# regicide211212/multi-style-transfer-gan

Hardware: AMD Instinct MI355X
Metric: train-step images/sec (fwd+bwd+loss), 256x256 batch32 (higher is better)
Workload: dtype f32; 1 GPU; config 3: reference CycleGAN train_step (2x EnhancedGenerator + 2x EnhancedDiscriminator, channels=16, num_transformer_blocks=0), 32 image pairs/GPU at 256x256, fwd+bwd+loss+Adam; per_gpu_batch=32, size=256, channels=16, parallelism=dp1, collective=none, losses_finite=True

## Files before the change

multi-style-transfer-gan_amd/mstg_hip/csrc/common.h:

```cpp
#pragma once
#include <hip/hip_runtime.h>
#include <stdint.h>
#include <stdio.h>
#include <string.h>

#include "mstg_hip.h"

typedef float f32x4 __attribute__((ext_vector_type(4)));
typedef float f32x2 __attribute__((ext_vector_type(2)));

namespace mstg {

extern thread_local char g_last_error[256];
inline int fail_launch(hipError_t e, const char* what) {
    snprintf(g_last_error, sizeof(g_last_error), "%s: %s", what, hipGetErrorString(e));
    return MSTG_E_LAUNCH;
}
inline int fail_arg(int code, const char* what) {
    snprintf(g_last_error, sizeof(g_last_error), "%s", what);
    return code;
}
#define MSTG_CHECK_LAUNCH(what)                                   \
    do {                                                          \
        hipError_t e__ = hipGetLastError();                       \
        if (e__ != hipSuccess) return mstg::fail_launch(e__, what); \
    } while (0)

extern bool g_prof_on;
void prof_begin(const void* host_fn, hipStream_t st);
void prof_end(hipStream_t st);
#define MSTG_LAUNCH(kern, grid, block, lds, st, ...)                               \
    do {                                                                           \
        const bool prof__ = mstg::g_prof_on;                                       \
        if (prof__) mstg::prof_begin((const void*)(kern), (hipStream_t)(st));      \
        hipLaunchKernelGGL(kern, grid, block, lds, st, __VA_ARGS__);               \
        if (prof__) mstg::prof_end((hipStream_t)(st));                             \
    } while (0)

extern thread_local bool t_ws_packed;
#define MSTG_PACK_LAUNCH(...)                      \
    do {                                           \
        if (!mstg::t_ws_packed) MSTG_LAUNCH(__VA_ARGS__); \
    } while (0)

enum EnvKnob {
    ENV_ATTN_BLK4, ENV_ATTN_BLK64, ENV_WGRAD_1X1, ENV_WGRAD_TS_MAXCH, ENV_WGRAD_PLAIN, ENV_WGRAD_OLD, ENV_NO_DPACK, ENV_IGEMM,
    ENV_STREAM, ENV_PF, ENV_WGLOB, ENV_HEAVY_PER_CU, ENV_DBG, ENV_DBG_LDS_KB, ENV_MS_WGRAD_PACKED, ENV_MS_FWD4, ENV_NO_PACK_CACHE,
    ENV_P32, ENV_P32_TH, ENV_P32_WLDS, ENV_P32_DBG, ENV_P32_OCC, ENV_ATTN_REG, ENV_NFW_ADAPT, ENV_BSUMS_ALL, ENV_ATTN_BIG32, ENV_NORM_WGS,
    ENV_CONV_IMG, ENV_COUNT
};
const char* env_get(EnvKnob k);

int cu_count();
struct OccCache {
    const void* kern = nullptr;
    size_t lds = 0;
    int occ = 1;
};
int persistent_occupancy(OccCache& c, const void* kern, size_t lds);

constexpr int WAVE = 64;

__device__ __forceinline__ f32x4 mfma16(float a, float b, f32x4 c) {
    return __builtin_amdgcn_mfma_f32_16x16x4f32(a, b, c, 0, 0, 0);
}

__device__ __forceinline__ float wave_sum(float v) {
#pragma unroll
    for (int o = 32; o > 0; o >>= 1) v += __shfl_xor(v, o, 64);
    return v;
}

__device__ __forceinline__ float apply_act(float v, int act) {
    switch (act) {
        case MSTG_ACT_RELU: return v > 0.f ? v : 0.f;
        case MSTG_ACT_LEAKY02: return v > 0.f ? v : 0.2f * v;
        case MSTG_ACT_TANH: return tanhf(v);
        case MSTG_ACT_GELU: return 0.5f * v * (1.f + erff(v * 0.70710678118654752f));
        default: return v;
    }
}
__device__ __forceinline__ float act_grad(float v, int act) {
    switch (act) {
        case MSTG_ACT_RELU: return v > 0.f ? 1.f : 0.f;
        case MSTG_ACT_LEAKY02: return v > 0.f ? 1.f : 0.2f;
        case MSTG_ACT_TANH: return 1.f - v * v;
        case MSTG_ACT_GELU: return 0.5f * (1.f + erff(v * 0.70710678118654752f)) + v * 0.3989422804014327f * expf(-0.5f * v * v);
        default: return 1.f;
    }
}

__device__ __forceinline__ int xcd_swizzle(int bid, int nblk) {
    const int q = nblk >> 3, r = nblk & 7, xcd = bid & 7, k = bid >> 3;
    return (xcd < r ? xcd * (q + 1) : r * (q + 1) + (xcd - r) * q) + k;
}


__host__ __device__ __forceinline__ unsigned magic_u32(unsigned d) { return 0xFFFFFFFFu / d + 1u; }

template <int NB>
__device__ __forceinline__ void stage_window_batch(const float* __restrict__ img, float* __restrict__ lds, int total, int e0, int cols,
                                                   int nq, unsigned m_cols, unsigned m_nq, int y0, int x0, int H, int W, int ctot,
                                                   int nq_valid, int ckp, int tid, int rowpad) {
    f32x4 v[NB];
    int dst[NB];
    bool ok[NB];
#pragma unroll
    for (int k = 0; k < NB; ++k) {
        const int e = e0 + 256 * k + tid;
        const int p = nq == 1 ? e : (int)__umulhi((unsigned)e, m_nq);
        const int q = e - p * nq;
        const int r = (int)__umulhi((unsigned)p, m_cols), c = p - r * cols;
        const int iy = y0 + r, ix = x0 + c;
        ok[k] = e < total && (unsigned)iy < (unsigned)H && (unsigned)ix < (unsigned)W && q < nq_valid;
        const unsigned off = ok[k] ? (unsigned)(iy * W + ix) * (unsigned)ctot + 4u * q : 0u;
        v[k] = *reinterpret_cast<const f32x4*>(img + off);
        dst[k] = e < total ? p * ckp + 4 * q + r * rowpad : -1;
    }
#pragma unroll
    for (int k = 0; k < NB; ++k)
        if (dst[k] >= 0) *reinterpret_cast<f32x4*>(&lds[dst[k]]) = ok[k] ? v[k] : f32x4{0.f, 0.f, 0.f, 0.f};
}

__device__ __forceinline__ void stage_window(const float* __restrict__ img, float* __restrict__ lds, int rows, int cols, int nq,
                                             unsigned m_cols, unsigned m_nq, int y0, int x0, int H, int W, int ctot, int nq_valid,
                                             int ckp, int tid, int rowpad = 0) {
    const int total = rows * cols * nq;
    int e0 = 0;
    for (; e0 + 1024 < total; e0 += 2048)
        stage_window_batch<8>(img, lds, total, e0, cols, nq, m_cols, m_nq, y0, x0, H, W, ctot, nq_valid, ckp, tid, rowpad);
    for (; e0 < total; e0 += 1024)
        stage_window_batch<4>(img, lds, total, e0, cols, nq, m_cols, m_nq, y0, x0, H, W, ctot, nq_valid, ckp, tid, rowpad);
}

__device__ __forceinline__ void stage_window_c4(const float* __restrict__ img, float* __restrict__ lds, int rows, int cols,
                                                unsigned m_cols, int y0, int x0, int H, int W, unsigned sy, unsigned sx, unsigned sc,
                                                int nch, int tid) {
    const int total = rows * cols;
    for (int e0 = 0; e0 < total; e0 += 1024) {
        f32x4 v[4];
        bool ok[4];
#pragma unroll
        for (int k = 0; k < 4; ++k) {
            const int e = e0 + 256 * k + tid;
            const int r = (int)__umulhi((unsigned)e, m_cols), c = e - r * cols;
            const int iy = y0 + r, ix = x0 + c;
            ok[k] = e < total && (unsigned)iy < (unsigned)H && (unsigned)ix < (unsigned)W;
            const unsigned off = ok[k] ? (unsigned)iy * sy + (unsigned)ix * sx : 0u;
#pragma unroll
            for (int ch = 0; ch < 4; ++ch) v[k][ch] = img[off + (ch < nch ? ch * sc : 0u)];
        }
#pragma unroll
        for (int k = 0; k < 4; ++k) {
            const int e = e0 + 256 * k + tid;
            if (e < total) {
                f32x4 w = {0.f, 0.f, 0.f, 0.f};
#pragma unroll
                for (int ch = 0; ch < 4; ++ch)
                    if (ok[k] && ch < nch) w[ch] = v[k][ch];
                *reinterpret_cast<f32x4*>(&lds[e * 4]) = w;
            }
        }
    }
}

inline int cdiv(int a, int b) { return (a + b - 1) / b; }
inline size_t cdivz(size_t a, size_t b) { return (a + b - 1) / b; }

}
```

multi-style-transfer-gan_amd/mstg_hip/csrc/norm.hip:

```cpp
#include "common.h"
#include <stdlib.h>

namespace mstg {

constexpr float NORM_EPS = 1e-5f;

struct NormGeom {
    int N, HW, C, split, chunk;
};

static NormGeom norm_geom(int N, int HW, int C) {
    NormGeom g;
    g.N = N; g.HW = HW; g.C = C;
    int wgs = 1024;
    { const char* e = env_get(ENV_NORM_WGS); if (e && atoi(e) >= 64) wgs = atoi(e); }
    int split = wgs / (N > 0 ? N : 1);
    if (split < 1) split = 1;
    const int maxsplit = cdiv(HW, 256);
    if (split > maxsplit) split = maxsplit;
    g.chunk = cdiv(HW, split);
    g.split = cdiv(HW, g.chunk);
    return g;
}

template <bool BWD>
__global__ __launch_bounds__(256) void norm_partial_kernel(const float* __restrict__ x, const float* __restrict__ dy,
                                                           const float* __restrict__ stats, const float* __restrict__ gamma,
                                                           const float* __restrict__ beta, float* __restrict__ partial,
                                                           NormGeom g, int act, int batch) {
    extern __shared__ __attribute__((aligned(16))) float red[];
    const int C = g.C, C4 = C >> 2, rows = 256 / C4;
    const int sp = blockIdx.x, n = blockIdx.y, tid = threadIdx.x;
    const int q = tid % C4, row = tid / C4;
    const int p0 = sp * g.chunk, p1 = min(g.HW, p0 + g.chunk);
    const float* xb = x + (size_t)n * g.HW * C;
    f32x4 s1 = {0.f, 0.f, 0.f, 0.f}, s2 = {0.f, 0.f, 0.f, 0.f};
    if (row < rows) {
        if (!BWD) {
            const f32x4 K = *reinterpret_cast<const f32x4*>((batch ? x : xb) + 4 * q);
            int p = p0 + row;
            constexpr int PX = 8;
            for (; p + (PX - 1) * rows < p1; p += PX * rows) {
                f32x4 v[PX];
#pragma unroll
                for (int k = 0; k < PX; ++k) v[k] = *reinterpret_cast<const f32x4*>(xb + (size_t)(p + k * rows) * C + 4 * q);
#pragma unroll
                for (int k = 0; k < PX; ++k) {
                    const f32x4 w = v[k] - K;
                    s1 += w;
                    s2 += w * w;
                }
            }
            for (; p < p1; p += rows) {
                const f32x4 v = *reinterpret_cast<const f32x4*>(xb + (size_t)p * C + 4 * q) - K;
                s1 += v;
                s2 += v * v;
            }
        } else {
            const float* st = stats + (size_t)(batch ? 0 : n) * C * 2;
            f32x4 mu, rs, ga = {1.f, 1.f, 1.f, 1.f}, be = {0.f, 0.f, 0.f, 0.f};
#pragma unroll
            for (int e = 0; e < 4; ++e) { mu[e] = st[(4 * q + e) * 2]; rs[e] = st[(4 * q + e) * 2 + 1]; }
            if (batch) { ga = *reinterpret_cast<const f32x4*>(gamma + 4 * q); be = *reinterpret_cast<const f32x4*>(beta + 4 * q); }
            const float* dyb = dy + (size_t)n * g.HW * C;
            int p = p0 + row;
            constexpr int PX = 8;
            for (; p + (PX - 1) * rows < p1; p += PX * rows) {
                f32x4 xv[PX], gv[PX];
#pragma unroll
                for (int k = 0; k < PX; ++k) {
                    xv[k] = *reinterpret_cast<const f32x4*>(xb + (size_t)(p + k * rows) * C + 4 * q);
                    gv[k] = *reinterpret_cast<const f32x4*>(dyb + (size_t)(p + k * rows) * C + 4 * q);
                }
#pragma unroll
                for (int k = 0; k < PX; ++k) {
                    const f32x4 xh = (xv[k] - mu) * rs;
                    f32x4 gg = gv[k];
#pragma unroll
                    for (int e = 0; e < 4; ++e) gg[e] *= act_grad(xh[e] * ga[e] + be[e], act);
                    s1 += gg;
                    s2 += gg * xh;
                }
            }
            for (; p < p1; p += rows) {
                const f32x4 xh = (*reinterpret_cast<const f32x4*>(xb + (size_t)p * C + 4 * q) - mu) * rs;
                f32x4 gg = *reinterpret_cast<const f32x4*>(dyb + (size_t)p * C + 4 * q);
#pragma unroll
                for (int e = 0; e < 4; ++e) gg[e] *= act_grad(xh[e] * ga[e] + be[e], act);
                s1 += gg;
                s2 += gg * xh;
            }
        }
        *reinterpret_cast<f32x4*>(&red[(row * 2 + 0) * C + 4 * q]) = s1;
        *reinterpret_cast<f32x4*>(&red[(row * 2 + 1) * C + 4 * q]) = s2;
    }
    __syncthreads();
    for (int e = tid; e < 2 * C; e += 256) {
        float acc = 0.f;
        for (int r = 0; r < rows; ++r) acc += red[r * 2 * C + e];
        partial[((size_t)n * g.split + sp) * 2 * C + e] = acc;
    }
}

template <bool BWD>
__global__ __launch_bounds__(256) void norm_apply_kernel(const float* __restrict__ x, const float* __restrict__ dy,
                                                         const float* __restrict__ residual, float* __restrict__ out,
                                                         float* __restrict__ stats, const float* __restrict__ gamma,
                                                         const float* __restrict__ beta, float* __restrict__ running_mean,
                                                         float* __restrict__ running_var, float* __restrict__ dgamma,
                                                         float* __restrict__ dbeta, const float* __restrict__ partial,
                                                         NormGeom g, int act, int batch, int psplit) {
    extern __shared__ __attribute__((aligned(16))) float sm[];
    const int C = g.C, C4 = C >> 2, rows = 256 / C4;
    const int sp = blockIdx.x, n = blockIdx.y, tid = threadIdx.x;
    const float cnt = batch ? (float)g.N * (float)g.HW : (float)g.HW;
    for (int c = tid; c < C; c += 256) {
        float t1 = 0.f, t2 = 0.f;
        if (batch != 2 && batch != 3) {
            const int nb = batch ? 0 : n, ne = batch ? g.N : n + 1;
            for (int nn = nb; nn < ne; ++nn) {
                const float* pp = partial + (size_t)nn * psplit * 2 * C + c;
                int s = 0;
                for (; s + 8 <= psplit; s += 8) {
                    float a[8], b[8];
#pragma unroll
                    for (int k = 0; k < 8; ++k) {
                        a[k] = pp[(size_t)(s + k) * 2 * C];
                        b[k] = pp[(size_t)(s + k) * 2 * C + C];
                    }
#pragma unroll
                    for (int k = 0; k < 8; ++k) {
                        t1 += a[k];
                        t2 += b[k];
                    }
                }
                for (; s < psplit; ++s) {
                    t1 += pp[(size_t)s * 2 * C];
                    t2 += pp[(size_t)s * 2 * C + C];
                }
            }
        }
        if (!BWD) {
            float mean, rstd;
            if (batch == 2) {
                mean = running_mean[c];
                rstd = rsqrtf(running_var[c] + NORM_EPS);
            } else if (batch == 3) {
                mean = stats[((size_t)n * C + c) * 2];
                rstd = stats[((size_t)n * C + c) * 2 + 1];
            } else {
                const float K = (batch ? x : x + (size_t)n * g.HW * C)[c];
                const float e1 = t1 / cnt;
                float var = t2 / cnt - e1 * e1;
                var = var > 0.f ? var : 0.f;
                mean = K + e1;
                rstd = rsqrtf(var + NORM_EPS);
                if (batch == 1 && sp == 0 && n == 0) {
                    running_mean[c] = 0.9f * running_mean[c] + 0.1f * mean;
                    running_var[c] = 0.9f * running_var[c] + 0.1f * var * (cnt / fmaxf(cnt - 1.f, 1.f));
                }
            }
            if (batch != 3 && sp == 0 && (!batch || n == 0)) {
                stats[((size_t)(batch ? 0 : n) * C + c) * 2] = mean;
                stats[((size_t)(batch ? 0 : n) * C + c) * 2 + 1] = rstd;
            }
            const bool affine = batch == 1 || batch == 2;
            const float ga = affine ? gamma[c] : 1.f, be = affine ? beta[c] : 0.f;
            sm[c] = rstd * ga;
            sm[C + c] = be;
            sm[2 * C + c] = mean;
        } else {
            const float* st = stats + (size_t)(batch ? 0 : n) * C * 2;
            const float mu = st[c * 2], rs = st[c * 2 + 1];
            const float ga = batch ? gamma[c] : 1.f;
            const float m1 = batch == 2 ? 0.f : t1 / cnt, m2 = batch == 2 ? 0.f : t2 / cnt;
            if (batch == 1 && sp == 0 && n == 0) { dgamma[c] = t2; dbeta[c] = t1; }
            sm[c] = mu;
            sm[C + c] = rs;
            sm[2 * C + c] = m1;
            sm[3 * C + c] = m2;
            (void)ga;
        }
    }
    __syncthreads();
    const int q = tid % C4, row = tid / C4;
    if (row >= rows) return;
    const int p0 = sp * g.chunk, p1 = min(g.HW, p0 + g.chunk);
    const size_t base = (size_t)n * g.HW * C;
    if (!BWD) {
        const f32x4 A = *reinterpret_cast<const f32x4*>(&sm[4 * q]), B = *reinterpret_cast<const f32x4*>(&sm[C + 4 * q]);
        const f32x4 M = *reinterpret_cast<const f32x4*>(&sm[2 * C + 4 * q]);
        int p = p0 + row;
        constexpr int PX = 8;
        for (; p + (PX - 1) * rows < p1; p += PX * rows) {
            f32x4 v[PX], r[PX];
#pragma unroll
            for (int k = 0; k < PX; ++k) {
                const size_t o = base + (size_t)(p + k * rows) * C + 4 * q;
                v[k] = __builtin_nontemporal_load(reinterpret_cast<const f32x4*>(x + o));
                if (residual) r[k] = __builtin_nontemporal_load(reinterpret_cast<const f32x4*>(residual + o));
            }
#pragma unroll
            for (int k = 0; k < PX; ++k) {
                const size_t o = base + (size_t)(p + k * rows) * C + 4 * q;
                f32x4 w = (v[k] - M) * A + B;
#pragma unroll
                for (int e = 0; e < 4; ++e) w[e] = apply_act(w[e], act);
                if (residual) w += r[k];
                *reinterpret_cast<f32x4*>(out + o) = w;
            }
        }
        for (; p < p1; p += rows) {
            const size_t o = base + (size_t)p * C + 4 * q;
            f32x4 v = (*reinterpret_cast<const f32x4*>(x + o) - M) * A + B;
#pragma unroll
            for (int e = 0; e < 4; ++e) v[e] = apply_act(v[e], act);
            if (residual) v += *reinterpret_cast<const f32x4*>(residual + o);
            *reinterpret_cast<f32x4*>(out + o) = v;
        }
    } else {
        const f32x4 mu = *reinterpret_cast<const f32x4*>(&sm[4 * q]), rs = *reinterpret_cast<const f32x4*>(&sm[C + 4 * q]);
        const f32x4 m1 = *reinterpret_cast<const f32x4*>(&sm[2 * C + 4 * q]), m2 = *reinterpret_cast<const f32x4*>(&sm[3 * C + 4 * q]);
        f32x4 ga = {1.f, 1.f, 1.f, 1.f}, be = {0.f, 0.f, 0.f, 0.f};
        if (batch) { ga = *reinterpret_cast<const f32x4*>(gamma + 4 * q); be = *reinterpret_cast<const f32x4*>(beta + 4 * q); }
        int p = p0 + row;
        constexpr int PX = 8;
        for (; p + (PX - 1) * rows < p1; p += PX * rows) {
            f32x4 xv[PX], gv[PX];
#pragma unroll
            for (int k = 0; k < PX; ++k) {
                const size_t o = base + (size_t)(p + k * rows) * C + 4 * q;
                xv[k] = __builtin_nontemporal_load(reinterpret_cast<const f32x4*>(x + o));
                gv[k] = __builtin_nontemporal_load(reinterpret_cast<const f32x4*>(dy + o));
            }
#pragma unroll
            for (int k = 0; k < PX; ++k) {
                const size_t o = base + (size_t)(p + k * rows) * C + 4 * q;
                const f32x4 xh = (xv[k] - mu) * rs;
                f32x4 gg = gv[k];
#pragma unroll
                for (int e = 0; e < 4; ++e) gg[e] *= act_grad(xh[e] * ga[e] + be[e], act);
                *reinterpret_cast<f32x4*>(out + o) = rs * ga * (gg - m1 - xh * m2);
            }
        }
        for (; p < p1; p += rows) {
            const size_t o = base + (size_t)p * C + 4 * q;
            const f32x4 xh = (*reinterpret_cast<const f32x4*>(x + o) - mu) * rs;
            f32x4 gg = *reinterpret_cast<const f32x4*>(dy + o);
#pragma unroll
            for (int e = 0; e < 4; ++e) gg[e] *= act_grad(xh[e] * ga[e] + be[e], act);
            *reinterpret_cast<f32x4*>(out + o) = rs * ga * (gg - m1 - xh * m2);
        }
    }
}

__device__ __forceinline__ void norm_row_sums(const float* __restrict__ partial, int n, int split, int C, int groups, float* red, float& t1,
                                              float& t2) {
    const int tid = threadIdx.x, c = tid % C, grp = tid / C;
    t1 = t2 = 0.f;
    if (grp < groups) {
        const float* pp = partial + (size_t)n * split * 2 * C + c;
        int s = grp;
        for (; s + 7 * groups < split; s += 8 * groups) {
            float a[8], b[8];
#pragma unroll
            for (int k = 0; k < 8; ++k) {
                a[k] = pp[(size_t)(s + k * groups) * 2 * C];
                b[k] = pp[(size_t)(s + k * groups) * 2 * C + C];
            }
#pragma unroll
            for (int k = 0; k < 8; ++k) {
                t1 += a[k];
                t2 += b[k];
            }
        }
        for (; s < split; s += groups) {
            t1 += pp[(size_t)s * 2 * C];
            t2 += pp[(size_t)s * 2 * C + C];
        }
    }
    if (groups > 1) {
        if (grp < groups) {
            red[(grp * 2 + 0) * C + c] = t1;
            red[(grp * 2 + 1) * C + c] = t2;
        }
        __syncthreads();
        if (grp == 0) {
            t1 = t2 = 0.f;
            for (int k = 0; k < groups; ++k) {
                t1 += red[(k * 2 + 0) * C + c];
                t2 += red[(k * 2 + 1) * C + c];
            }
        }
    }
}

static int norm_groups(const NormGeom& g) { return g.split > 32 && g.C <= 128 ? 256 / g.C : 1; }
static int norm_row_threads(const NormGeom& g) { const int t = g.C * norm_groups(g); return t < 64 ? 64 : ((t + 63) / 64) * 64; }

__global__ void norm_stats_kernel(const float* __restrict__ x, const float* __restrict__ partial, float* __restrict__ stats, NormGeom g,
                                  int groups) {
    extern __shared__ __attribute__((aligned(16))) float red[];
    const int n = blockIdx.x, C = g.C;
    const float cnt = (float)g.HW;
    float t1, t2;
    norm_row_sums(partial, n, g.split, C, groups, red, t1, t2);
    if ((int)threadIdx.x < C) {
        const int c = threadIdx.x;
        const float K = x[(size_t)n * g.HW * C + c];
        const float e1 = t1 / cnt;
        float var = t2 / cnt - e1 * e1;
        var = var > 0.f ? var : 0.f;
        stats[((size_t)n * C + c) * 2] = K + e1;
        stats[((size_t)n * C + c) * 2 + 1] = rsqrtf(var + NORM_EPS);
    }
}

__global__ void norm_sums_kernel(const float* __restrict__ partial, float* __restrict__ sums, NormGeom g, int groups) {
    extern __shared__ __attribute__((aligned(16))) float red[];
    const int n = blockIdx.x, C = g.C;
    float t1, t2;
    norm_row_sums(partial, n, g.split, C, groups, red, t1, t2);
    if ((int)threadIdx.x < C) {
        sums[((size_t)n * 2 + 0) * C + threadIdx.x] = t1;
        sums[((size_t)n * 2 + 1) * C + threadIdx.x] = t2;
    }
}

static int norm_check(int N, int HW, int C) {
    if (N <= 0 || HW <= 0 || C <= 0) return fail_arg(MSTG_E_BADARG, "norm: empty tensor");
    if (C % 4 || C > 1024) return fail_arg(MSTG_E_ALIGN, "norm: C must be a multiple of 4 and <= 1024");
    return MSTG_OK;
}

}

using namespace mstg;

extern "C" size_t mstg_norm_workspace_bytes(int N, int HW, int C) {
    if (N <= 0 || HW <= 0 || C <= 0) return 0;
    const NormGeom g = norm_geom(N, HW, C);
    return ((size_t)N * g.split * 2 * C + (size_t)N * 2 * C) * sizeof(float);
}

extern "C" int mstg_norm_act_fwd(const float* x, const float* residual, float* y, float* stats, int N, int HW, int C, int act,
                                 int batch_stats, const float* gamma, const float* beta, float* running_mean,
                                 float* running_var, void* workspace, size_t workspace_bytes, void* stream) {
    if (int rc = norm_check(N, HW, C)) return rc;
    if (!x || !y || !stats || !workspace) return fail_arg(MSTG_E_BADARG, "norm_fwd: null pointer");
    if (batch_stats && (!gamma || !beta || !running_mean || !running_var)) return fail_arg(MSTG_E_BADARG, "norm_fwd: batch norm needs gamma/beta/running stats");
    if (act == MSTG_ACT_TANH) return fail_arg(MSTG_E_UNSUPPORTED, "norm_fwd: tanh epilogue not supported");
    const NormGeom g = norm_geom(N, HW, C);
    if (workspace_bytes < mstg_norm_workspace_bytes(N, HW, C)) return fail_arg(MSTG_E_WORKSPACE, "norm_fwd: workspace too small");
    hipStream_t st = (hipStream_t)stream;
    const int rows = 256 / (C / 4);
    dim3 grid(g.split, N);
    if (batch_stats != 2) {
        MSTG_LAUNCH((norm_partial_kernel<false>), grid, dim3(256), (size_t)rows * 2 * C * sizeof(float), st, x, nullptr, nullptr,
                           gamma, beta, (float*)workspace, g, act, batch_stats);
        MSTG_CHECK_LAUNCH("norm_partial_kernel");
    }
    if (batch_stats == 0 && g.split > 32) {
        const int groups = norm_groups(g);
        MSTG_LAUNCH(norm_stats_kernel, dim3(N), dim3(norm_row_threads(g)), (size_t)groups * 2 * C * sizeof(float), st, x,
                    (const float*)workspace, stats, g, groups);
        MSTG_CHECK_LAUNCH("norm_stats_kernel");
        MSTG_LAUNCH((norm_apply_kernel<false>), grid, dim3(256), (size_t)4 * C * sizeof(float), st, x, nullptr, residual, y, stats, nullptr,
                    nullptr, nullptr, nullptr, nullptr, nullptr, nullptr, g, act, 3, 0);
        MSTG_CHECK_LAUNCH("norm_apply_kernel");
        return MSTG_OK;
    }
    MSTG_LAUNCH((norm_apply_kernel<false>), grid, dim3(256), (size_t)4 * C * sizeof(float), st, x, nullptr, residual, y, stats,
                       gamma, beta, running_mean, running_var, nullptr, nullptr, (const float*)workspace, g, act, batch_stats, g.split);
    MSTG_CHECK_LAUNCH("norm_apply_kernel");
    return MSTG_OK;
}

extern "C" int mstg_norm_act_bwd(const float* x, const float* stats, const float* dy, float* dx, int N, int HW, int C, int act,
                                 int batch_stats, const float* gamma, const float* beta, float* dgamma, float* dbeta,
                                 void* workspace, size_t workspace_bytes, void* stream) {
    if (int rc = norm_check(N, HW, C)) return rc;
    if (!x || !stats || !dy || !dx || !workspace) return fail_arg(MSTG_E_BADARG, "norm_bwd: null pointer");
    if (batch_stats == 1 && (!gamma || !beta || !dgamma || !dbeta)) return fail_arg(MSTG_E_BADARG, "norm_bwd: batch norm needs gamma/beta/dgamma/dbeta");
    if (batch_stats == 2) return fail_arg(MSTG_E_UNSUPPORTED, "norm_bwd: eval-mode batch norm backward not implemented");
    const NormGeom g = norm_geom(N, HW, C);
    if (workspace_bytes < mstg_norm_workspace_bytes(N, HW, C)) return fail_arg(MSTG_E_WORKSPACE, "norm_bwd: workspace too small");
    hipStream_t st = (hipStream_t)stream;
    const int rows = 256 / (C / 4);
    dim3 grid(g.split, N);
    MSTG_LAUNCH((norm_partial_kernel<true>), grid, dim3(256), (size_t)rows * 2 * C * sizeof(float), st, x, dy, stats, gamma, beta,
                       (float*)workspace, g, act, batch_stats);
    MSTG_CHECK_LAUNCH("norm_partial_kernel<bwd>");
    if (batch_stats == 0 && g.split > 32) {
        const int groups = norm_groups(g);
        float* sums = (float*)workspace + (size_t)N * g.split * 2 * C;
        MSTG_LAUNCH(norm_sums_kernel, dim3(N), dim3(norm_row_threads(g)), (size_t)groups * 2 * C * sizeof(float), st, (const float*)workspace,
                    sums, g, groups);
        MSTG_CHECK_LAUNCH("norm_sums_kernel");
        MSTG_LAUNCH((norm_apply_kernel<true>), grid, dim3(256), (size_t)4 * C * sizeof(float), st, x, dy, nullptr, dx, const_cast<float*>(stats),
                    gamma, beta, nullptr, nullptr, dgamma, dbeta, (const float*)sums, g, act, batch_stats, 1);
        MSTG_CHECK_LAUNCH("norm_apply_kernel<bwd>");
        return MSTG_OK;
    }
    MSTG_LAUNCH((norm_apply_kernel<true>), grid, dim3(256), (size_t)4 * C * sizeof(float), st, x, dy, nullptr, dx,
                       const_cast<float*>(stats), gamma, beta, nullptr, nullptr, dgamma, dbeta, (const float*)workspace, g, act,
                       batch_stats, g.split);
    MSTG_CHECK_LAUNCH("norm_apply_kernel<bwd>");
    return MSTG_OK;
}

extern "C" int mstg_norm_stats(const float* x, float* stats, int N, int HW, int C, void* workspace, size_t workspace_bytes,
                               void* stream) {
    if (int rc = norm_check(N, HW, C)) return rc;
    if (!x || !stats || !workspace) return fail_arg(MSTG_E_BADARG, "norm_stats: null pointer");
    const NormGeom g = norm_geom(N, HW, C);
    if (workspace_bytes < mstg_norm_workspace_bytes(N, HW, C)) return fail_arg(MSTG_E_WORKSPACE, "norm_stats: workspace too small");
    hipStream_t st = (hipStream_t)stream;
    const int rows = 256 / (C / 4);
    MSTG_LAUNCH((norm_partial_kernel<false>), dim3(g.split, N), dim3(256), (size_t)rows * 2 * C * sizeof(float), st, x, nullptr,
                       nullptr, nullptr, nullptr, (float*)workspace, g, MSTG_ACT_NONE, 0);
    MSTG_CHECK_LAUNCH("norm_partial_kernel");
    const int groups = norm_groups(g);
    MSTG_LAUNCH(norm_stats_kernel, dim3(N), dim3(norm_row_threads(g)), (size_t)groups * 2 * C * sizeof(float), st, x, (const float*)workspace,
                stats, g, groups);
    MSTG_CHECK_LAUNCH("norm_stats_kernel");
    return MSTG_OK;
}

extern "C" int mstg_norm_bwd_apply(const float* x, const float* stats, const float* dy, const float* sums, int sums_split, float* dx,
                                   int N, int HW, int C, int act, void* stream) {
    if (int rc = norm_check(N, HW, C)) return rc;
    if (!x || !stats || !dy || !sums || !dx) return fail_arg(MSTG_E_BADARG, "norm_bwd_apply: null pointer");
    if (sums_split < 1) return fail_arg(MSTG_E_BADARG, "norm_bwd_apply: sums_split must be >= 1");
    const NormGeom g = norm_geom(N, HW, C);
    MSTG_LAUNCH((norm_apply_kernel<true>), dim3(g.split, N), dim3(256), (size_t)4 * C * sizeof(float), (hipStream_t)stream, x, dy,
                       nullptr, dx, const_cast<float*>(stats), nullptr, nullptr, nullptr, nullptr, nullptr, nullptr, sums, g, act, 0, sums_split);
    MSTG_CHECK_LAUNCH("norm_apply_kernel<bwd>");
    return MSTG_OK;
}

extern "C" int mstg_norm_apply_fwd(const float* x, const float* stats, const float* residual, float* y, int N, int HW, int C, int act,
                                   void* stream) {
    if (int rc = norm_check(N, HW, C)) return rc;
    if (!x || !stats || !y) return fail_arg(MSTG_E_BADARG, "norm_apply_fwd: null pointer");
    if (act == MSTG_ACT_TANH) return fail_arg(MSTG_E_UNSUPPORTED, "norm_apply_fwd: tanh epilogue not supported");
    const NormGeom g = norm_geom(N, HW, C);
    MSTG_LAUNCH((norm_apply_kernel<false>), dim3(g.split, N), dim3(256), (size_t)4 * C * sizeof(float), (hipStream_t)stream, x, nullptr,
                       residual, y, const_cast<float*>(stats), nullptr, nullptr, nullptr, nullptr, nullptr, nullptr, nullptr, g, act, 3, 0);
    MSTG_CHECK_LAUNCH("norm_apply_kernel");
    return MSTG_OK;
}
```

multi-style-transfer-gan_amd/mstg_hip/csrc/runtime.hip:

```cpp
#include <stdlib.h>

#include <cxxabi.h>

#include <mutex>
#include <string>
#include <vector>

#include "common.h"

namespace mstg {

thread_local char g_last_error[256] = "";
thread_local bool t_ws_packed = false;

static const char* const kEnvNames[ENV_COUNT] = {
    "MSTG_ATTN_BLK4", "MSTG_ATTN_BLK64", "MSTG_WGRAD_1X1", "MSTG_WGRAD_TS_MAXCH", "MSTG_WGRAD_PLAIN", "MSTG_WGRAD_OLD", "MSTG_NO_DPACK",
    "MSTG_IGEMM", "MSTG_STREAM", "MSTG_PF", "MSTG_WGLOB", "MSTG_HEAVY_PER_CU", "MSTG_DBG", "MSTG_DBG_LDS_KB", "MSTG_MS_WGRAD_PACKED",
    "MSTG_MS_FWD4", "MSTG_NO_PACK_CACHE", "MSTG_P32", "MSTG_P32_TH", "MSTG_P32_WLDS", "MSTG_P32_DBG", "MSTG_P32_OCC", "MSTG_ATTN_REG", "MSTG_NFW_ADAPT", "MSTG_BSUMS_ALL", "MSTG_ATTN_BIG32", "MSTG_NORM_WGS",
    "MSTG_CONV_IMG"};

struct EnvCache {
    char val[ENV_COUNT][32];
    bool set[ENV_COUNT];
    EnvCache() { refresh(); }
    void refresh() {
        for (int k = 0; k < ENV_COUNT; ++k) {
            const char* e = getenv(kEnvNames[k]);
            set[k] = e != nullptr;
            snprintf(val[k], sizeof(val[k]), "%s", e ? e : "");
        }
    }
};
static EnvCache g_env;

const char* env_get(EnvKnob k) { return g_env.set[k] ? g_env.val[k] : nullptr; }

int cu_count() {
    static int cus = 0;
    if (!cus) {
        int dev = 0;
        hipDeviceProp_t p;
        if (hipGetDevice(&dev) == hipSuccess && hipGetDeviceProperties(&p, dev) == hipSuccess) cus = p.multiProcessorCount;
        if (cus <= 0) cus = 256;
    }
    return cus;
}

int persistent_occupancy(OccCache& c, const void* kern, size_t lds) {
    if (c.kern != kern || c.lds != lds) {
        if (lds > 64 * 1024) (void)hipFuncSetAttribute(kern, hipFuncAttributeMaxDynamicSharedMemorySize, 160 * 1024);
        int nb = 1;
        if (hipOccupancyMaxActiveBlocksPerMultiprocessor(&nb, kern, 256, lds) != hipSuccess || nb < 1) nb = 1;
        c.occ = nb > 4 ? 4 : nb;
        c.kern = kern;
        c.lds = lds;
    }
    return c.occ;
}

bool g_prof_on = false;
struct ProfRec {
    const void* fn;
    hipStream_t st;
    hipEvent_t e0, e1;
};
static std::vector<ProfRec> g_prof;
static std::mutex g_prof_mu;
static thread_local int t_prof_open = -1;

void prof_begin(const void* fn, hipStream_t st) {
    ProfRec r{fn, st, nullptr, nullptr};
    if (hipEventCreate(&r.e0) != hipSuccess || hipEventCreate(&r.e1) != hipSuccess) return;
    (void)hipEventRecord(r.e0, st);
    std::lock_guard<std::mutex> lk(g_prof_mu);
    t_prof_open = (int)g_prof.size();
    g_prof.push_back(r);
}
void prof_end(hipStream_t st) {
    std::lock_guard<std::mutex> lk(g_prof_mu);
    if (t_prof_open < 0 || t_prof_open >= (int)g_prof.size()) return;
    (void)hipEventRecord(g_prof[t_prof_open].e1, st);
    t_prof_open = -1;
}
static void prof_clear() {
    for (auto& r : g_prof) {
        (void)hipEventDestroy(r.e0);
        (void)hipEventDestroy(r.e1);
    }
    g_prof.clear();
}

}

extern "C" const char* mstg_version(void) { return "mstg-hip 0.2.0 gfx950"; }
extern "C" const char* mstg_arch(void) { return "gfx950"; }
extern "C" const char* mstg_last_error(void) { return mstg::g_last_error; }
extern "C" void mstg_env_refresh(void) { mstg::g_env.refresh(); }

extern "C" int mstg_prof_enable(int on) {
    std::lock_guard<std::mutex> lk(mstg::g_prof_mu);
    if (on) mstg::prof_clear();
    mstg::g_prof_on = on != 0;
    return MSTG_OK;
}
extern "C" int mstg_prof_count(void) {
    std::lock_guard<std::mutex> lk(mstg::g_prof_mu);
    return (int)mstg::g_prof.size();
}
extern "C" int mstg_prof_get(int i, char* name, size_t name_cap, float* ms) {
    mstg::ProfRec r;
    {
        std::lock_guard<std::mutex> lk(mstg::g_prof_mu);
        if (i < 0 || i >= (int)mstg::g_prof.size() || !name || !ms || name_cap < 8) return mstg::fail_arg(MSTG_E_BADARG, "mstg_prof_get: bad index or buffer");
        r = mstg::g_prof[i];
    }
    hipError_t e = hipEventSynchronize(r.e1);
    if (e == hipSuccess) e = hipEventElapsedTime(ms, r.e0, r.e1);
    if (e != hipSuccess) return mstg::fail_launch(e, "mstg_prof_get");
    const char* mangled = hipKernelNameRefByPtr(r.fn, r.st);
    std::string nm = mangled ? mangled : "?";
    int status = 0;
    char* dem = mangled ? abi::__cxa_demangle(mangled, nullptr, nullptr, &status) : nullptr;
    if (dem && status == 0) nm = dem;
    free(dem);
    int depth = 0, cut = -1;
    for (int k = (int)nm.size() - 1; k >= 0; --k) {
        if (nm[k] == ')') ++depth;
        else if (nm[k] == '(' && --depth == 0) { cut = k; break; }
    }
    if (cut > 0) nm.resize(cut);
    if (nm.rfind("void ", 0) == 0) nm.erase(0, 5);
    if (nm.rfind("mstg::", 0) == 0) nm.erase(0, 6);
    snprintf(name, name_cap, "%s", nm.c_str());
    return MSTG_OK;
}
```

Before: 1711 images/sec.

## Fuse instance-norm stats and apply into one per-sample kernel for small planes

```diff
diff --git a/multi-style-transfer-gan_amd/mstg_hip/csrc/common.h b/multi-style-transfer-gan_amd/mstg_hip/csrc/common.h
--- a/multi-style-transfer-gan_amd/mstg_hip/csrc/common.h
+++ b/multi-style-transfer-gan_amd/mstg_hip/csrc/common.h
@@ -47,7 +47,7 @@
     ENV_ATTN_BLK4, ENV_ATTN_BLK64, ENV_WGRAD_1X1, ENV_WGRAD_TS_MAXCH, ENV_WGRAD_PLAIN, ENV_WGRAD_OLD, ENV_NO_DPACK, ENV_IGEMM,
     ENV_STREAM, ENV_PF, ENV_WGLOB, ENV_HEAVY_PER_CU, ENV_DBG, ENV_DBG_LDS_KB, ENV_MS_WGRAD_PACKED, ENV_MS_FWD4, ENV_NO_PACK_CACHE,
     ENV_P32, ENV_P32_TH, ENV_P32_WLDS, ENV_P32_DBG, ENV_P32_OCC, ENV_ATTN_REG, ENV_NFW_ADAPT, ENV_BSUMS_ALL, ENV_ATTN_BIG32, ENV_NORM_WGS,
-    ENV_CONV_IMG, ENV_COUNT
+    ENV_CONV_IMG, ENV_NORM_ONE_LAUNCH, ENV_COUNT
 };
 const char* env_get(EnvKnob k);
 
diff --git a/multi-style-transfer-gan_amd/mstg_hip/csrc/norm.hip b/multi-style-transfer-gan_amd/mstg_hip/csrc/norm.hip
--- a/multi-style-transfer-gan_amd/mstg_hip/csrc/norm.hip
+++ b/multi-style-transfer-gan_amd/mstg_hip/csrc/norm.hip
@@ -21,6 +21,110 @@
     g.chunk = cdiv(HW, split);
     g.split = cdiv(HW, g.chunk);
     return g;
+}
+
+
+__device__ __forceinline__ void norm_fwd_term(const f32x4 v, const f32x4 K, f32x4& s1, f32x4& s2) {
+    const f32x4 w = v - K;
+    s1 += w;
+    s2 += w * w;
+}
+
+__device__ __forceinline__ f32x4 norm_bwd_gg(const f32x4 xv, const f32x4 gv, const f32x4 mu, const f32x4 rs, const f32x4 ga, const f32x4 be,
+                                             int act, f32x4& xh) {
+    xh = (xv - mu) * rs;
+    f32x4 gg = gv;
+#pragma unroll
+    for (int e = 0; e < 4; ++e) gg[e] *= act_grad(xh[e] * ga[e] + be[e], act);
+    return gg;
+}
+__device__ __forceinline__ void norm_bwd_term(const f32x4 xv, const f32x4 gv, const f32x4 mu, const f32x4 rs, const f32x4 ga, const f32x4 be,
+                                              int act, f32x4& s1, f32x4& s2) {
+#pragma clang fp contract(off)
+    f32x4 xh;
+    const f32x4 gg = norm_bwd_gg(xv, gv, mu, rs, ga, be, act, xh);
+    s1 = s1 + gg;
+#pragma unroll
+    for (int e = 0; e < 4; ++e) s2[e] = __builtin_fmaf(gg[e], xh[e], s2[e]);
+}
+__device__ __forceinline__ f32x4 norm_bwd_dx(const f32x4 xv, const f32x4 gv, const f32x4 mu, const f32x4 rs, const f32x4 ga, const f32x4 be,
+                                             const f32x4 m1, const f32x4 m2, int act) {
+    f32x4 xh;
+    const f32x4 gg = norm_bwd_gg(xv, gv, mu, rs, ga, be, act, xh);
+    return rs * ga * (gg - m1 - xh * m2);
+}
+
+__device__ __forceinline__ f32x4 norm_fwd_y(const f32x4 v, const f32x4 M, const f32x4 A, const f32x4 B, int act) {
+    f32x4 w = (v - M) * A + B;
+#pragma unroll
+    for (int e = 0; e < 4; ++e) w[e] = apply_act(w[e], act);
+    return w;
+}
+
+template <bool BWD, int PX>
+__device__ __forceinline__ void norm_thread_sums(const float* __restrict__ xb, const float* __restrict__ dyb, const f32x4 a, const f32x4 b,
+                                                 const f32x4 ga, const f32x4 be, int act, int p0, int p1, int row, int rows, int C, int q,
+                                                 f32x4& s1, f32x4& s2) {
+    int p = p0 + row;
+    if (!BWD) {
+        for (; p + (PX - 1) * rows < p1; p += PX * rows) {
+            f32x4 v[PX];
+#pragma unroll
+            for (int k = 0; k < PX; ++k) v[k] = *reinterpret_cast<const f32x4*>(xb + (size_t)(p + k * rows) * C + 4 * q);
+#pragma unroll
+            for (int k = 0; k < PX; ++k) norm_fwd_term(v[k], a, s1, s2);
+        }
+        for (; p < p1; p += rows) norm_fwd_term(*reinterpret_cast<const f32x4*>(xb + (size_t)p * C + 4 * q), a, s1, s2);
+    } else {
+        for (; p + (PX - 1) * rows < p1; p += PX * rows) {
+            f32x4 xv[PX], gv[PX];
+#pragma unroll
+            for (int k = 0; k < PX; ++k) {
+                xv[k] = *reinterpret_cast<const f32x4*>(xb + (size_t)(p + k * rows) * C + 4 * q);
+                gv[k] = *reinterpret_cast<const f32x4*>(dyb + (size_t)(p + k * rows) * C + 4 * q);
+            }
+#pragma unroll
+            for (int k = 0; k < PX; ++k) norm_bwd_term(xv[k], gv[k], a, b, ga, be, act, s1, s2);
+        }
+        for (; p < p1; p += rows)
+            norm_bwd_term(*reinterpret_cast<const f32x4*>(xb + (size_t)p * C + 4 * q), *reinterpret_cast<const f32x4*>(dyb + (size_t)p * C + 4 * q),
+                          a, b, ga, be, act, s1, s2);
+    }
+}
+
+__device__ __forceinline__ float norm_rows_sum(const float* red, int rows, int C, int e) {
+    float acc = 0.f;
+    for (int r = 0; r < rows; ++r) acc += red[r * 2 * C + e];
+    return acc;
+}
+
+__device__ __forceinline__ void norm_splits_sum(const float* pp, int psplit, int C, float& t1, float& t2) {
+    int s = 0;
+    for (; s + 8 <= psplit; s += 8) {
+        float a[8], b[8];
+#pragma unroll
+        for (int k = 0; k < 8; ++k) {
+            a[k] = pp[(size_t)(s + k) * 2 * C];
+            b[k] = pp[(size_t)(s + k) * 2 * C + C];
+        }
+#pragma unroll
+        for (int k = 0; k < 8; ++k) {
+            t1 += a[k];
+            t2 += b[k];
+        }
+    }
+    for (; s < psplit; ++s) {
+        t1 += pp[(size_t)s * 2 * C];
+        t2 += pp[(size_t)s * 2 * C + C];
+    }
+}
+
+__device__ __forceinline__ void norm_mean_rstd(float t1, float t2, float cnt, float K, float& mean, float& rstd, float& var) {
+    const float e1 = t1 / cnt;
+    var = t2 / cnt - e1 * e1;
+    var = var > 0.f ? var : 0.f;
+    mean = K + e1;
+    rstd = rsqrtf(var + NORM_EPS);
 }
 
 template <bool BWD>
@@ -36,70 +140,23 @@
     const float* xb = x + (size_t)n * g.HW * C;
     f32x4 s1 = {0.f, 0.f, 0.f, 0.f}, s2 = {0.f, 0.f, 0.f, 0.f};
     if (row < rows) {
+        const f32x4 one = {1.f, 1.f, 1.f, 1.f}, zero = {0.f, 0.f, 0.f, 0.f};
         if (!BWD) {
             const f32x4 K = *reinterpret_cast<const f32x4*>((batch ? x : xb) + 4 * q);
-            int p = p0 + row;
-            constexpr int PX = 8;
-            for (; p + (PX - 1) * rows < p1; p += PX * rows) {
-                f32x4 v[PX];
-#pragma unroll
-                for (int k = 0; k < PX; ++k) v[k] = *reinterpret_cast<const f32x4*>(xb + (size_t)(p + k * rows) * C + 4 * q);
-#pragma unroll
-                for (int k = 0; k < PX; ++k) {
-                    const f32x4 w = v[k] - K;
-                    s1 += w;
-                    s2 += w * w;
-                }
-            }
-            for (; p < p1; p += rows) {
-                const f32x4 v = *reinterpret_cast<const f32x4*>(xb + (size_t)p * C + 4 * q) - K;
-                s1 += v;
-                s2 += v * v;
-            }
+            norm_thread_sums<false, 8>(xb, nullptr, K, zero, one, zero, act, p0, p1, row, rows, C, q, s1, s2);
         } else {
             const float* st = stats + (size_t)(batch ? 0 : n) * C * 2;
-            f32x4 mu, rs, ga = {1.f, 1.f, 1.f, 1.f}, be = {0.f, 0.f, 0.f, 0.f};
+            f32x4 mu, rs, ga = one, be = zero;
 #pragma unroll
             for (int e = 0; e < 4; ++e) { mu[e] = st[(4 * q + e) * 2]; rs[e] = st[(4 * q + e) * 2 + 1]; }
             if (batch) { ga = *reinterpret_cast<const f32x4*>(gamma + 4 * q); be = *reinterpret_cast<const f32x4*>(beta + 4 * q); }
-            const float* dyb = dy + (size_t)n * g.HW * C;
-            int p = p0 + row;
-            constexpr int PX = 8;
-            for (; p + (PX - 1) * rows < p1; p += PX * rows) {
-                f32x4 xv[PX], gv[PX];
-#pragma unroll
-                for (int k = 0; k < PX; ++k) {
-                    xv[k] = *reinterpret_cast<const f32x4*>(xb + (size_t)(p + k * rows) * C + 4 * q);
-                    gv[k] = *reinterpret_cast<const f32x4*>(dyb + (size_t)(p + k * rows) * C + 4 * q);
-                }
-#pragma unroll
-                for (int k = 0; k < PX; ++k) {
-                    const f32x4 xh = (xv[k] - mu) * rs;
-                    f32x4 gg = gv[k];
-#pragma unroll
-                    for (int e = 0; e < 4; ++e) gg[e] *= act_grad(xh[e] * ga[e] + be[e], act);
-                    s1 += gg;
-                    s2 += gg * xh;
-                }
-            }
-            for (; p < p1; p += rows) {
-                const f32x4 xh = (*reinterpret_cast<const f32x4*>(xb + (size_t)p * C + 4 * q) - mu) * rs;
-                f32x4 gg = *reinterpret_cast<const f32x4*>(dyb + (size_t)p * C + 4 * q);
-#pragma unroll
-                for (int e = 0; e < 4; ++e) gg[e] *= act_grad(xh[e] * ga[e] + be[e], act);
-                s1 += gg;
-                s2 += gg * xh;
-            }
+            norm_thread_sums<true, 8>(xb, dy + (size_t)n * g.HW * C, mu, rs, ga, be, act, p0, p1, row, rows, C, q, s1, s2);
         }
         *reinterpret_cast<f32x4*>(&red[(row * 2 + 0) * C + 4 * q]) = s1;
         *reinterpret_cast<f32x4*>(&red[(row * 2 + 1) * C + 4 * q]) = s2;
     }
     __syncthreads();
-    for (int e = tid; e < 2 * C; e += 256) {
-        float acc = 0.f;
-        for (int r = 0; r < rows; ++r) acc += red[r * 2 * C + e];
-        partial[((size_t)n * g.split + sp) * 2 * C + e] = acc;
-    }
+    for (int e = tid; e < 2 * C; e += 256) partial[((size_t)n * g.split + sp) * 2 * C + e] = norm_rows_sum(red, rows, C, e);
 }
 
 template <bool BWD>
@@ -118,27 +175,8 @@
         float t1 = 0.f, t2 = 0.f;
         if (batch != 2 && batch != 3) {
             const int nb = batch ? 0 : n, ne = batch ? g.N : n + 1;
-            for (int nn = nb; nn < ne; ++nn) {
-                const float* pp = partial + (size_t)nn * psplit * 2 * C + c;
-                int s = 0;
-                for (; s + 8 <= psplit; s += 8) {
-                    float a[8], b[8];
-#pragma unroll
-                    for (int k = 0; k < 8; ++k) {
-                        a[k] = pp[(size_t)(s + k) * 2 * C];
-                        b[k] = pp[(size_t)(s + k) * 2 * C + C];
-                    }
-#pragma unroll
-                    for (int k = 0; k < 8; ++k) {
-                        t1 += a[k];
-                        t2 += b[k];
-                    }
-                }
-                for (; s < psplit; ++s) {
-                    t1 += pp[(size_t)s * 2 * C];
-                    t2 += pp[(size_t)s * 2 * C + C];
-                }
-            }
+            for (int nn = nb; nn < ne; ++nn)
+                norm_splits_sum(partial + (size_t)nn * psplit * 2 * C + c, psplit, C, t1, t2);
         }
         if (!BWD) {
             float mean, rstd;
@@ -149,12 +187,8 @@
                 mean = stats[((size_t)n * C + c) * 2];
                 rstd = stats[((size_t)n * C + c) * 2 + 1];
             } else {
-                const float K = (batch ? x : x + (size_t)n * g.HW * C)[c];
-                const float e1 = t1 / cnt;
-                float var = t2 / cnt - e1 * e1;
-                var = var > 0.f ? var : 0.f;
-                mean = K + e1;
-                rstd = rsqrtf(var + NORM_EPS);
+                float var;
+                norm_mean_rstd(t1, t2, cnt, (batch ? x : x + (size_t)n * g.HW * C)[c], mean, rstd, var);
                 if (batch == 1 && sp == 0 && n == 0) {
                     running_mean[c] = 0.9f * running_mean[c] + 0.1f * mean;
                     running_var[c] = 0.9f * running_var[c] + 0.1f * var * (cnt / fmaxf(cnt - 1.f, 1.f));
@@ -203,18 +237,14 @@
 #pragma unroll
             for (int k = 0; k < PX; ++k) {
                 const size_t o = base + (size_t)(p + k * rows) * C + 4 * q;
-                f32x4 w = (v[k] - M) * A + B;
-#pragma unroll
-                for (int e = 0; e < 4; ++e) w[e] = apply_act(w[e], act);
+                f32x4 w = norm_fwd_y(v[k], M, A, B, act);
                 if (residual) w += r[k];
                 *reinterpret_cast<f32x4*>(out + o) = w;
             }
         }
         for (; p < p1; p += rows) {
             const size_t o = base + (size_t)p * C + 4 * q;
-            f32x4 v = (*reinterpret_cast<const f32x4*>(x + o) - M) * A + B;
-#pragma unroll
-            for (int e = 0; e < 4; ++e) v[e] = apply_act(v[e], act);
+            f32x4 v = norm_fwd_y(*reinterpret_cast<const f32x4*>(x + o), M, A, B, act);
             if (residual) v += *reinterpret_cast<const f32x4*>(residual + o);
             *reinterpret_cast<f32x4*>(out + o) = v;
         }
@@ -236,20 +266,13 @@
 #pragma unroll
             for (int k = 0; k < PX; ++k) {
                 const size_t o = base + (size_t)(p + k * rows) * C + 4 * q;
-                const f32x4 xh = (xv[k] - mu) * rs;
-                f32x4 gg = gv[k];
-#pragma unroll
-                for (int e = 0; e < 4; ++e) gg[e] *= act_grad(xh[e] * ga[e] + be[e], act);
-                *reinterpret_cast<f32x4*>(out + o) = rs * ga * (gg - m1 - xh * m2);
+                *reinterpret_cast<f32x4*>(out + o) = norm_bwd_dx(xv[k], gv[k], mu, rs, ga, be, m1, m2, act);
             }
         }
         for (; p < p1; p += rows) {
             const size_t o = base + (size_t)p * C + 4 * q;
-            const f32x4 xh = (*reinterpret_cast<const f32x4*>(x + o) - mu) * rs;
-            f32x4 gg = *reinterpret_cast<const f32x4*>(dy + o);
-#pragma unroll
-            for (int e = 0; e < 4; ++e) gg[e] *= act_grad(xh[e] * ga[e] + be[e], act);
-            *reinterpret_cast<f32x4*>(out + o) = rs * ga * (gg - m1 - xh * m2);
+            *reinterpret_cast<f32x4*>(out + o) = norm_bwd_dx(*reinterpret_cast<const f32x4*>(x + o), *reinterpret_cast<const f32x4*>(dy + o), mu, rs,
+                                                             ga, be, m1, m2, act);
         }
     }
 }
@@ -327,6 +350,135 @@
     }
 }
 
+constexpr int NORM_ONE_THREADS = 1024, NORM_ONE_VWG = NORM_ONE_THREADS / 256;
+constexpr int NORM_ONE_MAX_ROW_FLOATS = 4096;
+constexpr size_t NORM_ONE_PLANE_LIMIT = (size_t)128 * 1024;
+
+static size_t norm_one_lds_bytes(const NormGeom& g) {
+    return ((size_t)NORM_ONE_VWG * 2048 + (size_t)g.split * 2 * g.C + (size_t)4 * g.C) * sizeof(float);
+}
+
+static bool norm_one_launch(const NormGeom& g, int batch_stats) {
+    if (batch_stats != 0 || g.split > 32) return false;
+    if ((size_t)g.HW * g.C * sizeof(float) > NORM_ONE_PLANE_LIMIT || g.split * 2 * g.C > NORM_ONE_MAX_ROW_FLOATS) return false;
+    const char* e = env_get(ENV_NORM_ONE_LAUNCH);
+    return !(e && atoi(e) == 0);
+}
+
+template <bool BWD>
+__global__ __launch_bounds__(NORM_ONE_THREADS) void norm_one_kernel(const float* x, const float* dy, const float* residual, float* out,
+                                                                    float* stats, NormGeom g, int act) {
+    extern __shared__ __attribute__((aligned(16))) float sm[];
+    constexpr int NORM_ONE_PX = BWD ? 4 : 8;
+    const int C = g.C, C4 = C >> 2, rows = 256 / C4;
+    float* rowsum = sm + NORM_ONE_VWG * 2048;
+    float* coef = rowsum + g.split * 2 * C;
+    const int n = blockIdx.x, tid = threadIdx.x, vw = tid >> 8, vt = tid & 255;
+    float* red = sm + vw * 2048;
+    const float* xb = x + (size_t)n * g.HW * C;
+    const float* dyb = BWD ? dy + (size_t)n * g.HW * C : nullptr;
+    const float* st = stats + (size_t)n * C * 2;
+    const f32x4 one = {1.f, 1.f, 1.f, 1.f}, zero = {0.f, 0.f, 0.f, 0.f};
+    {
+        const int q = vt % C4, row = vt / C4;
+        f32x4 a = zero, b = zero;
+        if (row < rows) {
+            if (!BWD) {
+                a = *reinterpret_cast<const f32x4*>(xb + 4 * q);
+            } else {
+#pragma unroll
+                for (int e = 0; e < 4; ++e) { a[e] = st[(4 * q + e) * 2]; b[e] = st[(4 * q + e) * 2 + 1]; }
+            }
+        }
+        for (int sp0 = 0; sp0 < g.split; sp0 += NORM_ONE_VWG) {
+            const int sp = sp0 + vw;
+            if (sp < g.split && row < rows) {
+                const int p0 = sp * g.chunk, p1 = min(g.HW, p0 + g.chunk);
+                f32x4 s1 = zero, s2 = zero;
+                norm_thread_sums<BWD, NORM_ONE_PX>(xb, dyb, a, b, one, zero, act, p0, p1, row, rows, C, q, s1, s2);
+                *reinterpret_cast<f32x4*>(&red[(row * 2 + 0) * C + 4 * q]) = s1;
+                *reinterpret_cast<f32x4*>(&red[(row * 2 + 1) * C + 4 * q]) = s2;
+            }
+            __syncthreads();
+            if (sp < g.split)
+                for (int e = vt; e < 2 * C; e += 256) rowsum[sp * 2 * C + e] = norm_rows_sum(red, rows, C, e);
+            __syncthreads();
+        }
+    }
+    const float cnt = (float)g.HW;
+    for (int c = tid; c < C; c += NORM_ONE_THREADS) {
+        float t1 = 0.f, t2 = 0.f;
+        norm_splits_sum(rowsum + c, g.split, C, t1, t2);
+        if (!BWD) {
+            float mean, rstd, var;
+            norm_mean_rstd(t1, t2, cnt, xb[c], mean, rstd, var);
+            stats[((size_t)n * C + c) * 2] = mean;
+            stats[((size_t)n * C + c) * 2 + 1] = rstd;
+            coef[c] = rstd;
+            coef[C + c] = 0.f;
+            coef[2 * C + c] = mean;
+        } else {
+            coef[c] = st[c * 2];
+            coef[C + c] = st[c * 2 + 1];
+            coef[2 * C + c] = t1 / cnt;
+            coef[3 * C + c] = t2 / cnt;
+        }
+    }
+    __syncthreads();
+    const int arows = NORM_ONE_THREADS / C4, q = tid % C4, row = tid / C4;
+    if (row >= arows) return;
+    const size_t base = (size_t)n * g.HW * C;
+    const f32x4 c0 = *reinterpret_cast<const f32x4*>(&coef[4 * q]), c1 = *reinterpret_cast<const f32x4*>(&coef[C + 4 * q]);
+    const f32x4 c2 = *reinterpret_cast<const f32x4*>(&coef[2 * C + 4 * q]);
+    constexpr int PX = NORM_ONE_PX;
+    int p = row;
+    if (!BWD) {
+        for (; p + (PX - 1) * arows < g.HW; p += PX * arows) {
+            f32x4 v[PX], r[PX];
+#pragma unroll
+            for (int k = 0; k < PX; ++k) {
+                const size_t o = base + (size_t)(p + k * arows) * C + 4 * q;
+                v[k] = *reinterpret_cast<const f32x4*>(x + o);
+                if (residual) r[k] = __builtin_nontemporal_load(reinterpret_cast<const f32x4*>(residual + o));
+            }
+#pragma unroll
+            for (int k = 0; k < PX; ++k) {
+                const size_t o = base + (size_t)(p + k * arows) * C + 4 * q;
+                f32x4 w = norm_fwd_y(v[k], c2, c0, c1, act);
+                if (residual) w += r[k];
+                *reinterpret_cast<f32x4*>(out + o) = w;
+            }
+        }
+        for (; p < g.HW; p += arows) {
+            const size_t o = base + (size_t)p * C + 4 * q;
+            f32x4 w = norm_fwd_y(*reinterpret_cast<const f32x4*>(x + o), c2, c0, c1, act);
+            if (residual) w += *reinterpret_cast<const f32x4*>(residual + o);
+            *reinterpret_cast<f32x4*>(out + o) = w;
+        }
+    } else {
+        const f32x4 c3 = *reinterpret_cast<const f32x4*>(&coef[3 * C + 4 * q]);
+        for (; p + (PX - 1) * arows < g.HW; p += PX * arows) {
+            f32x4 xv[PX], gv[PX];
+#pragma unroll
+            for (int k = 0; k < PX; ++k) {
+                const size_t o = base + (size_t)(p + k * arows) * C + 4 * q;
+                xv[k] = *reinterpret_cast<const f32x4*>(x + o);
+                gv[k] = *reinterpret_cast<const f32x4*>(dy + o);
+            }
+#pragma unroll
+            for (int k = 0; k < PX; ++k) {
+                const size_t o = base + (size_t)(p + k * arows) * C + 4 * q;
+                *reinterpret_cast<f32x4*>(out + o) = norm_bwd_dx(xv[k], gv[k], c0, c1, one, zero, c2, c3, act);
+            }
+        }
+        for (; p < g.HW; p += arows) {
+            const size_t o = base + (size_t)p * C + 4 * q;
+            *reinterpret_cast<f32x4*>(out + o) = norm_bwd_dx(*reinterpret_cast<const f32x4*>(x + o), *reinterpret_cast<const f32x4*>(dy + o), c0, c1,
+                                                             one, zero, c2, c3, act);
+        }
+    }
+}
+
 static int norm_check(int N, int HW, int C) {
     if (N <= 0 || HW <= 0 || C <= 0) return fail_arg(MSTG_E_BADARG, "norm: empty tensor");
     if (C % 4 || C > 1024) return fail_arg(MSTG_E_ALIGN, "norm: C must be a multiple of 4 and <= 1024");
@@ -355,6 +507,11 @@
     hipStream_t st = (hipStream_t)stream;
     const int rows = 256 / (C / 4);
     dim3 grid(g.split, N);
+    if (norm_one_launch(g, batch_stats)) {
+        MSTG_LAUNCH((norm_one_kernel<false>), dim3(N), dim3(NORM_ONE_THREADS), norm_one_lds_bytes(g), st, x, nullptr, residual, y, stats, g, act);
+        MSTG_CHECK_LAUNCH("norm_one_kernel");
+        return MSTG_OK;
+    }
     if (batch_stats != 2) {
         MSTG_LAUNCH((norm_partial_kernel<false>), grid, dim3(256), (size_t)rows * 2 * C * sizeof(float), st, x, nullptr, nullptr,
                            gamma, beta, (float*)workspace, g, act, batch_stats);
@@ -388,6 +545,12 @@
     hipStream_t st = (hipStream_t)stream;
     const int rows = 256 / (C / 4);
     dim3 grid(g.split, N);
+    if (norm_one_launch(g, batch_stats)) {
+        MSTG_LAUNCH((norm_one_kernel<true>), dim3(N), dim3(NORM_ONE_THREADS), norm_one_lds_bytes(g), st, x, dy, nullptr, dx,
+                    const_cast<float*>(stats), g, act);
+        MSTG_CHECK_LAUNCH("norm_one_kernel<bwd>");
+        return MSTG_OK;
+    }
     MSTG_LAUNCH((norm_partial_kernel<true>), grid, dim3(256), (size_t)rows * 2 * C * sizeof(float), st, x, dy, stats, gamma, beta,
                        (float*)workspace, g, act, batch_stats);
     MSTG_CHECK_LAUNCH("norm_partial_kernel<bwd>");
diff --git a/multi-style-transfer-gan_amd/mstg_hip/csrc/runtime.hip b/multi-style-transfer-gan_amd/mstg_hip/csrc/runtime.hip
--- a/multi-style-transfer-gan_amd/mstg_hip/csrc/runtime.hip
+++ b/multi-style-transfer-gan_amd/mstg_hip/csrc/runtime.hip
@@ -17,7 +17,7 @@
     "MSTG_ATTN_BLK4", "MSTG_ATTN_BLK64", "MSTG_WGRAD_1X1", "MSTG_WGRAD_TS_MAXCH", "MSTG_WGRAD_PLAIN", "MSTG_WGRAD_OLD", "MSTG_NO_DPACK",
     "MSTG_IGEMM", "MSTG_STREAM", "MSTG_PF", "MSTG_WGLOB", "MSTG_HEAVY_PER_CU", "MSTG_DBG", "MSTG_DBG_LDS_KB", "MSTG_MS_WGRAD_PACKED",
     "MSTG_MS_FWD4", "MSTG_NO_PACK_CACHE", "MSTG_P32", "MSTG_P32_TH", "MSTG_P32_WLDS", "MSTG_P32_DBG", "MSTG_P32_OCC", "MSTG_ATTN_REG", "MSTG_NFW_ADAPT", "MSTG_BSUMS_ALL", "MSTG_ATTN_BIG32", "MSTG_NORM_WGS",
-    "MSTG_CONV_IMG"};
+    "MSTG_CONV_IMG", "MSTG_NORM_ONE_LAUNCH"};
 
 struct EnvCache {
     char val[ENV_COUNT][32];
```

After: 1709 images/sec. Within noise of the previous version (-0.1%).
